# ayushpradhan-dev/robust-speech-analysis-framework

Measured on AMD Instinct MI355X. Metric: audio-seconds processed/sec (extract+CNN-LSTM fwd), higher is better.
Workload: dtype f32

## Files before the change

### robust_speech_analysis_framework_amd/csrc/gemm_f16x3.hip

```cpp
#include <algorithm>
#include <type_traits>

#include "gemm_f16x3.h"

namespace rsaf {

using f32x16 = __attribute__((ext_vector_type(16))) float;
using f16x8 = __attribute__((ext_vector_type(8))) _Float16;
typedef __attribute__((address_space(3))) void* lds_ptr3;
typedef const __attribute__((address_space(1))) void* glb_ptr3;

__device__ __forceinline__ unsigned short f16_bits(_Float16 h) { return __builtin_bit_cast(unsigned short, h); }

__device__ __forceinline__ void split2(float xs, unsigned short& h, unsigned short& l) {
    const _Float16 hh = (_Float16)xs;
    const _Float16 ll = (_Float16)(xs - (float)hh);
    h = f16_bits(hh);
    l = f16_bits(ll);
}

template <int TM_, int TN_, int WM_, int WN_, int NST_, int WGS_>
struct H3Cfg {
    static constexpr int TM = TM_, TN = TN_, WM = WM_, WN = WN_, NST = NST_, WGS = WGS_;
    static constexpr int BM = 32 * TM * WM, BN = 32 * TN * WN, BK = 16, NPL = 2;
    static constexpr int THREADS = 64 * WM * WN;
    static constexpr int A_PLANE = BM * BK, B_PLANE = BN * BK;
    static constexpr int STAGE = NPL * (A_PLANE + B_PLANE);
    static constexpr int A_INSTR = BM / 32, B_INSTR = BN / 32;
    static constexpr int PATCH_BYTES = WM * WN * 32 * 36 * 4;
    static constexpr int TAB_BYTES = 2 * (BM + BN) * 4 + 2 * BM * 4;
    static constexpr bool PATCH_IN_STAGE2 = BM > 256;
    static_assert(!PATCH_IN_STAGE2 || STAGE * 2 >= PATCH_BYTES, "stage 2 must hold the epilogue patches");
    static constexpr int LDS_BYTES = NST * STAGE * 2 + (PATCH_IN_STAGE2 ? 0 : PATCH_BYTES) + TAB_BYTES;
};

#if defined(__HIP_DEVICE_COMPILE__)
#define H3_OPAQUE(SP, LB) asm volatile("" : "+s"(SP), "+v"(LB))
#else
#define H3_OPAQUE(SP, LB) (void)0
#endif
#define H3_ADDR(UNIFORM_BASE, LANE_BYTES)                                                                      \
    ({                                                                                                         \
        const char* sp_ = reinterpret_cast<const char*>(UNIFORM_BASE);                                         \
        unsigned lb_ = (LANE_BYTES);                                                                           \
        H3_OPAQUE(sp_, lb_);                                                                                   \
        (glb_ptr3)(sp_ + lb_);                                                                                 \
    })

template <class CFG, int ACT, bool OUT_F32, bool OUT_PLANES, bool HAS_R, bool ROWTAB = false>
__global__ __launch_bounds__(CFG::THREADS, CFG::WGS * CFG::THREADS / 256) void gemm_f16x3_kernel(const GemmH3Params p) {
    extern __shared__ __attribute__((aligned(1024))) unsigned short smem3[];
    constexpr int BM = CFG::BM, BN = CFG::BN, BK = CFG::BK, STAGE = CFG::STAGE, NST = CFG::NST, NPL = CFG::NPL;
    constexpr int TM = CFG::TM, TN = CFG::TN, NW = CFG::WM * CFG::WN;
    constexpr int A_PLANE = CFG::A_PLANE, B_PLANE = CFG::B_PLANE;

    const int tid = threadIdx.x, lane = tid & 63, wave = __builtin_amdgcn_readfirstlane(tid >> 6), l31 = lane & 31, h = lane >> 5;
    const unsigned total_tiles = (unsigned)p.nwg * (unsigned)p.nz;
    const int wm0 = (wave / CFG::WN) * (32 * TM), wn0 = (wave % CFG::WN) * (32 * TN);

    struct Tile { int m0, n0, Mz, z, z1, z2; int64_t coff, aoff, boff; unsigned t; bool valid; };
    auto next_valid = [&](unsigned t) {
        Tile T;
        T.valid = false;
        for (; t < total_tiles; t += gridDim.x) {
            const H3Tile W = h3_tile_at(p, (int)t);
            T.m0 = W.tm * BM; T.n0 = W.tn * BN; T.z = W.z; T.z1 = W.z1; T.z2 = W.z2;
            T.Mz = p.ztab ? (int)p.ztab[2 * W.z1] : p.M;
            if (T.m0 < T.Mz) {
                T.coff = p.ztab ? p.ztab[2 * W.z1 + 1] : -1;
                T.aoff = W.z1 * p.sA + W.z2 * p.sA2 + (int64_t)T.m0 * (p.a_panel ? 16 : p.lda);
                T.boff = W.z2 * p.sB2 + (int64_t)T.n0 * (p.b_panel ? 16 : p.ldb);
                T.t = t; T.valid = true;
                break;
            }
        }
        return T;
    };

    constexpr int NI = CFG::A_INSTR + CFG::B_INSTR;
    constexpr int IPW = (NI + NW - 1) / NW;
    constexpr int A_SLOTS = CFG::A_INSTR / NW;
    constexpr int LAST_LIVE = NI - NW * (IPW - 1);
    static_assert(CFG::A_INSTR % NW == 0, "a slot is an A or a B instruction for every wave alike");
    static_assert(LAST_LIVE == NW || LAST_LIVE <= NW / 2, "the waves of group B have the same number of DMA instructions");
    const bool last_live = LAST_LIVE == NW || wave < LAST_LIVE;
#define H3_LIVE(i) ((i) < IPW - 1 || last_live)
    const char* src[IPW][NPL];
    unsigned voff[IPW];
    int ldsoff[IPW];
    int pc = 0;
    const H3KStep a_step = h3_kstep(p.a_panel ? (int64_t)(p.a_panel_rows > 0 ? p.a_panel_rows : p.M) * 16 : 16, p.a_tap_panels, 2);
    const int64_t b_step = 2 * (p.b_panel ? (int64_t)(p.b_panel_rows > 0 ? p.b_panel_rows : p.N) * 16 : 16);
#pragma unroll
    for (int i = 0; i < IPW; ++i) {
        const int jj = i < A_SLOTS ? wave + NW * i : wave + NW * i - CFG::A_INSTR;
        ldsoff[i] = i < A_SLOTS ? jj * 512 : NPL * A_PLANE + jj * 512;
    }
    auto set_tile = [&](const Tile& T) {
        pc = 0;
#pragma unroll
        for (int i = 0; i < IPW; ++i) {
            const bool isA = i < A_SLOTS;
            const int jj = isA ? wave + NW * i : wave + NW * i - CFG::A_INSTR;
            const int row = 32 * jj + (lane >> 1);
            const int dch = (lane & 1) ^ ((row >> 3) & 1);
            const int rr = isA ? ((T.m0 + row < T.Mz) ? row : T.Mz - 1 - T.m0)
                               : ((T.n0 + row < p.N) ? row : p.N - 1 - T.n0);
            const int64_t rs = isA ? (p.a_panel ? 16 : p.lda) : (p.b_panel ? 16 : p.ldb);
            voff[i] = 2u * ((unsigned)rr * (unsigned)rs + 8u * dch);
            const unsigned short* base = isA ? p.A + T.aoff : p.B + T.boff;
#pragma unroll
            for (int pl = 0; pl < NPL; ++pl)
                src[i][pl] = reinterpret_cast<const char*>(base + pl * (isA ? p.a_plane : p.b_plane));
        }
    };
#define H3_DMA(ST)                                                                                              \
    do {                                                                                                        \
        _Pragma("unroll") for (int i = 0; i < IPW; ++i) {                                                       \
            if (H3_LIVE(i)) {                                                                                   \
                _Pragma("unroll") for (int pl = 0; pl < NPL; ++pl)                                              \
                    __builtin_amdgcn_global_load_lds(H3_ADDR(src[i][pl], voff[i]),                              \
                        (lds_ptr3)(smem3 + (ST) + ldsoff[i] + pl * (i < A_SLOTS ? A_PLANE : B_PLANE)), 16, 0, 0); \
            }                                                                                                   \
        }                                                                                                       \
    } while (0)
#define H3_ADVANCE()                                                                                            \
    do {                                                                                                        \
        const int64_t a_inc_ = h3_kstep_next(a_step, pc);                                                       \
        _Pragma("unroll") for (int i = 0; i < IPW; ++i)                                                         \
            _Pragma("unroll") for (int pl = 0; pl < NPL; ++pl) src[i][pl] += i < A_SLOTS ? a_inc_ : b_step;     \
    } while (0)
    const int nk = p.K / BK;
    auto prefetch = [&](const Tile& T) {
        set_tile(T);
        H3_DMA(0);
        if (nk > 1) {
            H3_ADVANCE();
            H3_DMA(STAGE);
            H3_ADVANCE();
        }
    };

    static_assert(NST == 3 && TM % 2 == 0, "the staggered loop needs three stages and an even number of m-tiles");
    const int grpB = wave >= NW / 2 ? 1 : 0;
    constexpr int NDMA_B = NPL * (LAST_LIVE == NW ? IPW : IPW - 1);
    constexpr int HM = TM / 2;
    constexpr int PATCH_LD = 36;
    float* patch = reinterpret_cast<float*>(smem3 + (CFG::PATCH_IN_STAGE2 ? 2 : NST) * STAGE) + wave * (32 * PATCH_LD);

    constexpr int TPT = (BM + BN + CFG::THREADS - 1) / CFG::THREADS;
    float* tab0 = reinterpret_cast<float*>(smem3 + NST * STAGE) + (CFG::PATCH_IN_STAGE2 ? 0 : NW * (32 * PATCH_LD));
    float* tab1 = tab0 + (BM + BN);
    int* tab_slot = reinterpret_cast<int*>(tab1 + (BM + BN));
    int* tab_dest = tab_slot + BM;
    float e0[TPT], e1[TPT];
    int e_slot[TPT], e_dest[TPT];
    auto load_epi = [&](const Tile& T) {
#pragma unroll
        for (int u = 0; u < TPT; ++u) {
            const int i = tid + u * CFG::THREADS;
            e0[u] = 1.0f; e1[u] = 0.0f;
            if (i < BM) {
                const int row = T.m0 + i < T.Mz ? T.m0 + i : T.Mz - 1;
                if (ROWTAB) {
                    const int2 rt = reinterpret_cast<const int2*>(p.row_tab)[row];
                    e_slot[u] = rt.x; e_dest[u] = rt.y;
                    e0[u] = p.a_scale[rt.x];
                    e1[u] = (OUT_PLANES && p.Cp) ? p.c_scale[rt.x] : 1.0f;
                } else {
                    e0[u] = p.a_scale[(int64_t)T.z1 * p.a_scale_zs + (int64_t)row * p.a_scale_ms];
                    e1[u] = (OUT_PLANES && p.Cp) ? p.c_scale[(int64_t)T.z1 * p.c_scale_zs + (int64_t)row * p.c_scale_ms] : 1.0f;
                }
            } else if (i < BM + BN) {
                const int col = T.n0 + i - BM;
                e0[u] = col < p.N ? p.b_scale[T.z2 * p.sBias2 + col] : 1.0f;
                e1[u] = (p.bias && col < p.N) ? p.bias[T.z2 * p.sBias2 + col] : 0.0f;
            }
        }
    };
    Tile cur = next_valid(blockIdx.x);
    if (!cur.valid) return;
    load_epi(cur);
    prefetch(cur);

    while (true) {
    const Tile nxt = next_valid(cur.t + gridDim.x);
    f32x16 acc[TM][TN];
#pragma unroll
    for (int i = 0; i < TM; ++i)
#pragma unroll
        for (int j = 0; j < TN; ++j)
#pragma unroll
            for (int e = 0; e < 16; ++e) acc[i][j][e] = 0.0f;

    int s0 = 0, s1 = STAGE, s2 = 2 * STAGE;
    auto ktile = [&](auto refill_c, auto grpb_c) __attribute__((always_inline)) {
        constexpr bool REFILL = decltype(refill_c)::value, GRPB = decltype(grpb_c)::value;
        if (!GRPB) asm volatile("s_waitcnt vmcnt(0)" ::: "memory");
        __builtin_amdgcn_s_barrier();
        asm volatile("" ::: "memory");
        const unsigned short* img = smem3 + s0;
        f16x8 bf[TN][NPL];
#pragma unroll
        for (int nt = 0; nt < TN; ++nt) {
            const int row = wn0 + nt * 32 + l31;
            const int off = row * BK + ((h ^ ((row >> 3) & 1)) << 3);
#pragma unroll
            for (int pl = 0; pl < NPL; ++pl) bf[nt][pl] = *reinterpret_cast<const f16x8*>(&img[NPL * A_PLANE + pl * B_PLANE + off]);
        }
        if (REFILL) {
            H3_DMA(GRPB ? s2 : s1);
            H3_ADVANCE();
        }
        f16x8 afp[NPL];
#pragma unroll
        for (int mt = 0; mt < TM; ++mt) {
            f16x8 af[NPL];
            if (mt == HM) {
#pragma unroll
                for (int pl = 0; pl < NPL; ++pl) af[pl] = afp[pl];
            } else {
                const int row = wm0 + mt * 32 + l31;
                const int off = row * BK + ((h ^ ((row >> 3) & 1)) << 3);
#pragma unroll
                for (int pl = 0; pl < NPL; ++pl) af[pl] = *reinterpret_cast<const f16x8*>(&img[pl * A_PLANE + off]);
            }
            if (mt == HM - 1) {
                const int row = wm0 + HM * 32 + l31;
                const int off = row * BK + ((h ^ ((row >> 3) & 1)) << 3);
#pragma unroll
                for (int pl = 0; pl < NPL; ++pl) afp[pl] = *reinterpret_cast<const f16x8*>(&img[pl * A_PLANE + off]);
            }
#pragma unroll
            for (int nt = 0; nt < TN; ++nt) {
                f32x16 c = acc[mt][nt];
                c = __builtin_amdgcn_mfma_f32_32x32x16_f16(af[1], bf[nt][0], c, 0, 0, 0);
                c = __builtin_amdgcn_mfma_f32_32x32x16_f16(af[0], bf[nt][1], c, 0, 0, 0);
                c = __builtin_amdgcn_mfma_f32_32x32x16_f16(af[0], bf[nt][0], c, 0, 0, 0);
                acc[mt][nt] = c;
            }
            if (mt == HM - 1) {
                if (GRPB) asm volatile("s_waitcnt vmcnt(%0)" ::"n"(REFILL ? NDMA_B : 0) : "memory");
                __builtin_amdgcn_s_barrier();
                asm volatile("" ::: "memory");
            }
        }
        const int s_ = s0; s0 = s1; s1 = s2; s2 = s_;
    };
    constexpr std::true_type YES{};
    constexpr std::false_type NO{};
    asm volatile("s_waitcnt vmcnt(0)" ::: "memory");
    if (!grpB) {
        ktile(NO, NO);
        for (int kt = 1; kt < nk - 1; ++kt) ktile(YES, NO);
        if (nk > 1) ktile(NO, NO);
        __builtin_amdgcn_s_barrier();
    } else {
        __builtin_amdgcn_s_barrier();
        for (int kt = 0; kt < nk - 2; ++kt) ktile(YES, YES);
        if (nk > 1) ktile(NO, YES);
        ktile(NO, YES);
    }

    const Tile done = cur;
    constexpr int CW = (OUT_PLANES && !OUT_F32) ? 8 : 4, LPR = 32 / CW, RPI = 64 / LPR, NQ = 32 / RPI;
    const int lr = lane / LPR, c4 = CW * (lane % LPR);
    float4 r4[4];
    auto load_r = [&](int mt, int nt) {
        const int tn = done.n0 + wn0 + nt * 32, tm = done.m0 + wm0 + mt * 32;
        const float* Rt = p.R + (int64_t)done.z * p.sR + (int64_t)tm * p.ldr + tn + c4;
#pragma unroll
        for (int q = 0; q < 4; ++q) {
            const bool ok = (tn + c4) < p.N && (tm + 8 * q + lr) < done.Mz;
            r4[q] = (ok && p.R) ? *reinterpret_cast<const float4*>(Rt + (8 * q + lr) * (int)p.ldr) : make_float4(0.f, 0.f, 0.f, 0.f);
        }
    };
#pragma unroll
    for (int u = 0; u < TPT; ++u) {
        const int i = tid + u * CFG::THREADS;
        if (i < BM + BN) { tab0[i] = e0[u]; tab1[i] = e1[u]; }
        if (ROWTAB && i < BM) { tab_slot[i] = e_slot[u]; tab_dest[i] = e_dest[u]; }
    }
    if (HAS_R) load_r(0, 0);

    __syncthreads();
    cur = nxt;
    if (cur.valid) {
        prefetch(cur);
        load_epi(cur);
    }

    {
    const int m0 = done.m0, n0 = done.n0, Mz = done.Mz;
    const int64_t z = done.z, z1 = done.z1, z2 = done.z2;
    static_assert(!HAS_R || CW == 4, "the residual comes with the fp32 output");
#pragma unroll
    for (int mt = 0; mt < TM; ++mt) {
        const int tm = m0 + wm0 + mt * 32;
        float asi[NQ], csc[NQ], row_amax[NQ];
        int drow[NQ];
#pragma unroll
        for (int q = 0; q < NQ; ++q) {
            asi[q] = p.alpha * pow2_inverse(tab0[wm0 + mt * 32 + RPI * q + lr]);
            csc[q] = tab1[wm0 + mt * 32 + RPI * q + lr];
            row_amax[q] = 0.0f;
            drow[q] = ROWTAB ? tab_dest[wm0 + mt * 32 + RPI * q + lr] : tm + RPI * q + lr;
        }
#pragma unroll
        for (int nt = 0; nt < TN; ++nt) {
            const int tn = n0 + wn0 + nt * 32;
            const int gc = tn + c4;
            const bool c_ok = gc < p.N;
            float bsi[CW], bias4[CW];
#pragma unroll
            for (int j4 = 0; j4 < CW / 4; ++j4) {
                const float4 bs4 = *reinterpret_cast<const float4*>(tab0 + BM + wn0 + nt * 32 + c4 + 4 * j4);
                const float4 bi4 = *reinterpret_cast<const float4*>(tab1 + BM + wn0 + nt * 32 + c4 + 4 * j4);
                bsi[4 * j4] = pow2_inverse(bs4.x); bsi[4 * j4 + 1] = pow2_inverse(bs4.y);
                bsi[4 * j4 + 2] = pow2_inverse(bs4.z); bsi[4 * j4 + 3] = pow2_inverse(bs4.w);
                bias4[4 * j4] = bi4.x; bias4[4 * j4 + 1] = bi4.y; bias4[4 * j4 + 2] = bi4.z; bias4[4 * j4 + 3] = bi4.w;
            }
            constexpr int LAST = TM * TN - 1;
            const int sub = mt * TN + nt;
#pragma unroll
            for (int e = 0; e < 16; ++e) patch[(4 * h + (e & 3) + 8 * (e >> 2)) * PATCH_LD + l31] = acc[mt][nt][e];
            __builtin_amdgcn_fence(__ATOMIC_RELEASE, "wavefront");
            __builtin_amdgcn_wave_barrier();
            __builtin_amdgcn_fence(__ATOMIC_ACQUIRE, "wavefront");
            float v[NQ][CW];
#pragma unroll
            for (int q = 0; q < NQ; ++q)
#pragma unroll
                for (int j4 = 0; j4 < CW / 4; ++j4) {
                    const float4 t4 = *reinterpret_cast<const float4*>(patch + (RPI * q + lr) * PATCH_LD + c4 + 4 * j4);
                    v[q][4 * j4] = t4.x; v[q][4 * j4 + 1] = t4.y; v[q][4 * j4 + 2] = t4.z; v[q][4 * j4 + 3] = t4.w;
                }
            __builtin_amdgcn_wave_barrier();
#pragma unroll
            for (int q = 0; q < NQ; ++q) {
                float rv[4] = {0.f, 0.f, 0.f, 0.f};
                if (HAS_R) { rv[0] = r4[q % 4].x; rv[1] = r4[q % 4].y; rv[2] = r4[q % 4].z; rv[3] = r4[q % 4].w; }
#pragma unroll
                for (int j = 0; j < CW; ++j) {
                    float y = v[q][j] * (asi[q] * bsi[j]) + bias4[j];
                    if (HAS_R) y += rv[j % 4];
                    if (ACT == ACT_SILU) y = y / (1.0f + expf(-y));
                    v[q][j] = y;
                    if (ACT == ACT_GELU && (j & 1)) {
                        const gelu_f32x2 g2 = gelu_pair(gelu_f32x2{v[q][j - 1], v[q][j]});
                        v[q][j - 1] = g2.x; v[q][j] = g2.y;
                    }
                    if (ACT != ACT_NONE && (j & 3) == 3) __builtin_amdgcn_sched_barrier(0);
                }
            }
            if (HAS_R && sub < LAST) load_r((sub + 1) / TN, (sub + 1) % TN);
#pragma unroll
            for (int q = 0; q < NQ; ++q) {
                const int row = drow[q];
                const bool ok = c_ok && tm + RPI * q + lr < Mz && (!ROWTAB || row >= 0);
                if (p.amax_out && ok && gc >= p.amax_col_min) {
#pragma unroll
                    for (int j = 0; j < CW; ++j) row_amax[q] = fmaxf(row_amax[q], fabsf(v[q][j]));
                }
                if (ok) {
                    if (OUT_F32 && p.C) *reinterpret_cast<float4*>(p.C + (done.coff >= 0 ? done.coff : z1 * p.sC) + z2 * p.sC2 + (int64_t)row * p.ldc + gc) =
                        make_float4(v[q][0], v[q][1], v[q][2], v[q][3]);
                    if (OUT_PLANES && p.Cp) {
                        const float cs = csc[q];
                        unsigned short hh[CW], ll[CW];
#pragma unroll
                        for (int j = 0; j < CW; ++j) split2(v[q][j] * cs, hh[j], ll[j]);
                        unsigned short* Pt = p.cp_panel ? p.Cp + (int64_t)(gc >> 4) * ((int64_t)p.M * 16) + (int64_t)row * 16 + (gc & 15)
                                                        : p.Cp + z * p.sCp + (int64_t)row * p.ldcp + gc;
                        if (CW == 8) {
                            *reinterpret_cast<uint4*>(Pt) = make_uint4(hh[0] | ((unsigned)hh[1] << 16), hh[2] | ((unsigned)hh[3] << 16),
                                                                      hh[4 % CW] | ((unsigned)hh[5 % CW] << 16), hh[6 % CW] | ((unsigned)hh[7 % CW] << 16));
                            *reinterpret_cast<uint4*>(Pt + p.c_plane) = make_uint4(ll[0] | ((unsigned)ll[1] << 16), ll[2] | ((unsigned)ll[3] << 16),
                                                                                  ll[4 % CW] | ((unsigned)ll[5 % CW] << 16), ll[6 % CW] | ((unsigned)ll[7 % CW] << 16));
                        } else {
                            *reinterpret_cast<uint2*>(Pt) = make_uint2(hh[0] | ((unsigned)hh[1] << 16), hh[2] | ((unsigned)hh[3] << 16));
                            *reinterpret_cast<uint2*>(Pt + p.c_plane) = make_uint2(ll[0] | ((unsigned)ll[1] << 16), ll[2] | ((unsigned)ll[3] << 16));
                        }
                    }
                }
            }
        }
        if (p.amax_out) {
#pragma unroll
            for (int q = 0; q < NQ; ++q) {
                const int row = tm + RPI * q + lr;
                const bool r_ok = row < Mz && (!ROWTAB || drow[q] >= 0);
                const int slot = !r_ok ? -1 : ROWTAB ? tab_slot[wm0 + mt * 32 + RPI * q + lr]
                                                     : (int)(z1 * p.amax_zs) + (p.amax_row_slot ? p.amax_row_slot[row] : 0);
                unsigned long long todo = __ballot(r_ok);
                while (todo) {
                    const int first = __ffsll((long long)todo) - 1;
                    const int s0 = __shfl(slot, first, 64);
                    const bool mine = r_ok && slot == s0;
                    float mx = mine ? row_amax[q] : 0.0f;
#pragma unroll
                    for (int o = 32; o >= 1; o >>= 1) mx = fmaxf(mx, __shfl_xor(mx, o, 64));
                    if (lane == first && mx > 0.0f) atomicMax(p.amax_out + s0, __float_as_uint(mx));
                    todo &= ~__ballot(mine);
                }
            }
        }
    }
    }
    if (!cur.valid) break;
    }
#undef H3_DMA
#undef H3_ADVANCE
#undef H3_LIVE
}

__global__ __launch_bounds__(256) void f16x2_row_scales_kernel(const float* __restrict__ src, int64_t rows, int K, int64_t ld,
                                                               float* __restrict__ scale, float* __restrict__ norm2,
                                                               unsigned* __restrict__ stat_max) {
    const int64_t row = (int64_t)blockIdx.x * 4 + (threadIdx.x >> 6);
    if (row >= rows) return;
    const int lane = threadIdx.x & 63;
    const float* x = src + row * ld;
    float mx = 0.0f;
    double ss = 0.0;
    for (int k = lane; k < K; k += 64) {
        const float v = x[k];
        mx = fmaxf(mx, fabsf(v));
        ss += (double)v * (double)v;
    }
#pragma unroll
    for (int o = 32; o >= 1; o >>= 1) mx = fmaxf(mx, __shfl_xor(mx, o, 64));
    ss = wave_sum_f64(ss);
    if (lane == 0) {
        scale[row] = f16x2_scale_for_bound(mx);
        const float nn = (float)sqrt(ss) * 1.0000002f;
        if (norm2) norm2[row] = nn;
        if (stat_max) {
            atomicMax(stat_max + 0, __float_as_uint(nn));
            atomicMax(stat_max + 1, __float_as_uint(mx));
        }
    }
}

__global__ __launch_bounds__(256) void split_f16x2_kernel(const float* __restrict__ src, int64_t rows, int K, int64_t ld,
                                                          const float* __restrict__ scale, int scale_stride,
                                                          unsigned short* __restrict__ planes, int64_t plane_stride, int panels) {
    const int64_t row = (int64_t)blockIdx.x * 256 + threadIdx.x;
    if (row >= rows) return;
    const int kb = blockIdx.y;
    const float s = scale[row * scale_stride];
    const float4* s4 = reinterpret_cast<const float4*>(src + row * ld + 16 * kb);
    unsigned short h[16], l[16];
#pragma unroll
    for (int q = 0; q < 4; ++q) {
        const float4 v = s4[q];
        split2(v.x * s, h[4 * q], l[4 * q]); split2(v.y * s, h[4 * q + 1], l[4 * q + 1]);
        split2(v.z * s, h[4 * q + 2], l[4 * q + 2]); split2(v.w * s, h[4 * q + 3], l[4 * q + 3]);
    }
    auto pk = [](const unsigned short* s_, int o) {
        return make_uint4(s_[o] | ((unsigned)s_[o + 1] << 16), s_[o + 2] | ((unsigned)s_[o + 3] << 16),
                          s_[o + 4] | ((unsigned)s_[o + 5] << 16), s_[o + 6] | ((unsigned)s_[o + 7] << 16));
    };
    unsigned short* d = panels ? planes + (int64_t)kb * rows * 16 + row * 16 : planes + row * K + 16 * kb;
    *reinterpret_cast<uint4*>(d) = pk(h, 0); *reinterpret_cast<uint4*>(d + 8) = pk(h, 8);
    *reinterpret_cast<uint4*>(d + plane_stride) = pk(l, 0); *reinterpret_cast<uint4*>(d + plane_stride + 8) = pk(l, 8);
}

__global__ __launch_bounds__(256) void scale_from_bound_kernel(const unsigned* __restrict__ amax_bits, int64_t n,
                                                               const float* __restrict__ factor_dev, float factor_host,
                                                               const float* __restrict__ add_dev, float* __restrict__ scale) {
    const int64_t i = (int64_t)blockIdx.x * 256 + threadIdx.x;
    if (i >= n) return;
    const float f = factor_host * (factor_dev ? *factor_dev : 1.0f);
    const float a = add_dev ? *add_dev : 0.0f;
    scale[i] = f16x2_scale_for_bound(__uint_as_float(amax_bits[i]) * f + a);
}

int launch_f16x2_row_scales(const float* src, int64_t rows, int K, int64_t ld, float* scale, float* norm2, unsigned* stat_max,
                            hipStream_t stream) {
    RSAF_CHECK_ARG(rows >= 0 && K >= 0 && ld >= K, "bad shape");
    if (rows == 0) return RSAF_OK;
    RSAF_CHECK_ARG(src && scale, "NULL pointer");
    RSAF_CHECK_ARG((rows + 3) / 4 <= 0x7fffffffLL, "too many rows");
    hipLaunchKernelGGL(f16x2_row_scales_kernel, dim3((unsigned)((rows + 3) / 4)), dim3(256), 0, stream, src, rows, K, ld, scale, norm2,
                       stat_max);
    RSAF_CHECK_HIP(hipGetLastError());
    return RSAF_OK;
}

int launch_split_f16x2(const float* src, int64_t rows, int K, int64_t ld, const float* scale, int scale_stride, uint16_t* planes,
                       int64_t plane_stride, int panels, hipStream_t stream) {
    RSAF_CHECK_ARG(rows >= 0 && K >= 0 && K % 16 == 0 && ld % 4 == 0 && ld >= K, "K must be a non-negative multiple of 16, ld a multiple of 4");
    if (rows == 0 || K == 0) return RSAF_OK;
    RSAF_CHECK_ARG(src && planes && scale, "NULL pointer");
    RSAF_CHECK_ARG(plane_stride % 8 == 0 && K / 16 <= 65535 && (scale_stride == 0 || scale_stride == 1),
                   "plane stride must be a multiple of 8 elements; at most 65535 panels; scale stride 0 or 1");
    RSAF_CHECK_ARG((reinterpret_cast<uintptr_t>(src) & 15) == 0 && (reinterpret_cast<uintptr_t>(planes) & 15) == 0, "16-byte alignment");
    ProfScope prof("split_f16x2", stream, 0.0, 8.0 * (double)rows * K);
    hipLaunchKernelGGL(split_f16x2_kernel, dim3((unsigned)((rows + 255) / 256), (unsigned)(K / 16)), dim3(256), 0, stream, src, rows, K,
                       ld, scale, scale_stride, reinterpret_cast<unsigned short*>(planes), plane_stride, panels);
    RSAF_CHECK_HIP(hipGetLastError());
    return RSAF_OK;
}

int launch_scale_from_bound(const unsigned* amax_bits, int64_t n, const float* factor_dev, float factor_host, const float* add_dev,
                            float* scale, hipStream_t stream) {
    if (n <= 0) return RSAF_OK;
    RSAF_CHECK_ARG(amax_bits && scale, "NULL pointer");
    hipLaunchKernelGGL(scale_from_bound_kernel, dim3((unsigned)((n + 255) / 256)), dim3(256), 0, stream, amax_bits, n, factor_dev,
                       factor_host, add_dev, scale);
    RSAF_CHECK_HIP(hipGetLastError());
    return RSAF_OK;
}

int launch_gemm_f16x3(const GemmH3Params& p, hipStream_t stream, const char* tag) {
    RSAF_CHECK_ARG(p.M >= 0 && p.N >= 0 && p.K >= 0 && p.nz >= 0, "negative dimension");
    if (p.M == 0 || p.N == 0 || p.nz == 0) return RSAF_OK;
    RSAF_CHECK_ARG(p.A && p.B && (p.C || p.Cp), "NULL operand");
    RSAF_CHECK_ARG(p.a_scale && p.b_scale && (!p.Cp || p.c_scale), "every plane operand needs its scales");
    RSAF_CHECK_ARG(p.K % 16 == 0 && p.K >= 16, "K must be a positive multiple of 16");
    RSAF_CHECK_ARG(p.N % 16 == 0, "N must be a multiple of 16 (16-byte epilogue stores)");
    RSAF_CHECK_ARG(p.ldc % 8 == 0 && p.ldcp % 8 == 0 && p.ldr % 4 == 0 && p.c_plane % 8 == 0 && p.sC % 4 == 0 && p.sCp % 8 == 0 &&
                   p.sR % 4 == 0 && p.sC2 % 4 == 0, "ldc / ldr / output strides must keep 16-byte alignment");
    RSAF_CHECK_ARG(p.lda % 8 == 0 && p.ldb % 8 == 0 && p.a_plane % 8 == 0 && p.b_plane % 8 == 0 && p.sA % 8 == 0 && p.sA2 % 8 == 0 &&
                   p.sB2 % 8 == 0, "lda, ldb, the plane strides and the batch strides must be multiples of 8 elements");
    RSAF_CHECK_ARG((reinterpret_cast<uintptr_t>(p.A) & 15) == 0 && (reinterpret_cast<uintptr_t>(p.B) & 15) == 0 &&
                   (reinterpret_cast<uintptr_t>(p.b_scale) & 15) == 0 && p.sBias2 % 4 == 0, "A, B and b_scale must be 16-byte aligned");
    RSAF_CHECK_ARG(!p.R || p.ldr > 0, "residual needs ldr");
    RSAF_CHECK_ARG(p.act >= 0 && p.act <= 2, "act must be 0 (none), 1 (gelu) or 2 (silu)");
    RSAF_CHECK_ARG(p.nz <= 65535, "at most 65535 batches per launch");
    RSAF_CHECK_ARG(!p.cp_panel || p.nz == 1, "the panel layout of the plane output is for unbatched operands");
    RSAF_CHECK_ARG(!p.a_panel || p.nz == 1 || p.a_panel_rows > 0, "a batched A in panels needs a_panel_rows");
    RSAF_CHECK_ARG(p.a_tap_panels == 0 || (p.a_panel && p.a_panel_rows > 0 && p.a_tap_panels > 0 && (p.K / 16) % p.a_tap_panels == 0),
                   "a_tap_panels: A in panels with a_panel_rows, K = taps x a_tap_panels x 16");
    RSAF_CHECK_ARG(p.ldc < (1 << 24) && p.ldcp < (1 << 24) && p.ldr < (1 << 24), "leading dimensions must be below 2^24");
    RSAF_CHECK_ARG(!p.R || p.C, "the residual comes with the fp32 output");
    RSAF_CHECK_ARG(!p.row_tab || (p.nz == 1 && !p.ztab && p.nz2 <= 1 && !p.cp_panel && !p.a_panel && !p.amax_row_slot),
                   "a row table: one batch, row-major A and plane output, no ztab / amax_row_slot");
    RSAF_CHECK_ARG(p.nz2 <= 1 || (p.C && !p.Cp && !p.R && (!p.a_panel || p.a_panel_rows > 0) && p.nz % p.nz2 == 0),
                   "two-level batches: fp32 output only, no residual, A row-major or panels with a_panel_rows, nz a multiple of nz2");
    ProfScope prof(tag ? tag : "gemm_f16x3", stream, 2.0 * p.M * (double)p.N * p.K * p.nz, 0.0);
    using CfgA = H3Cfg<4, 2, 2, 4, 3, 1>;
    using CfgN = H3Cfg<2, 1, 4, 2, 3, 1>;
    using CfgM = H3Cfg<4, 2, 4, 2, 3, 1>;
#define H3_LAUNCH_CFG(CFG, ACT, F32, PL, HR, ...)                                                                       \
    do {                                                                                                                \
        RSAF_CHECK_HIP(hipFuncSetAttribute((const void*)gemm_f16x3_kernel<CFG, ACT, F32, PL, HR, ##__VA_ARGS__>,         \
                                           hipFuncAttributeMaxDynamicSharedMemorySize, CFG::LDS_BYTES));                 \
        RSAF_CHECK_ARG(h3_grid_fill(pp, CFG::BM, CFG::BN), "too many tiles");                                           \
        const int64_t tiles = (int64_t)pp.nwg * pp.nz;                                                                  \
        hipLaunchKernelGGL((gemm_f16x3_kernel<CFG, ACT, F32, PL, HR, ##__VA_ARGS__>),                                    \
                           dim3((unsigned)std::min<int64_t>(tiles, persistent_wgs)), dim3(CFG::THREADS), CFG::LDS_BYTES, stream, pp); \
    } while (0)
#define H3_LAUNCH(ACT, F32, PL, HR, ...)                                                                                \
    do {                                                                                                                \
        if (p.N <= 64) H3_LAUNCH_CFG(CfgN, ACT, F32, PL, HR, ##__VA_ARGS__);                                             \
        else H3_LAUNCH_CFG(CfgA, ACT, F32, PL, HR, ##__VA_ARGS__);                                                       \
    } while (0)
#define H3_LAUNCH3(ACT, F32, PL, HR)                                                                                    \
    do {                                                                                                                \
        if (p.N <= 64) H3_LAUNCH_CFG(CfgN, ACT, F32, PL, HR);                                                            \
        else if (p.N <= 128) H3_LAUNCH_CFG(CfgM, ACT, F32, PL, HR);                                                      \
        else H3_LAUNCH_CFG(CfgA, ACT, F32, PL, HR);                                                                      \
    } while (0)
    GemmH3Params pp = p;
    if (pp.group_m <= 0) pp.group_m = 2;
    int persistent_wgs = 256;
    {
        int dev = 0, cus = 0;
        if (hipGetDevice(&dev) == hipSuccess && hipDeviceGetAttribute(&cus, hipDeviceAttributeMultiprocessorCount, dev) == hipSuccess && cus > 0)
            persistent_wgs = cus;
    }
    const bool f32o = p.C != nullptr, plo = p.Cp != nullptr, hr = p.R != nullptr;
    if (p.row_tab) {
        if (p.act == ACT_GELU && !f32o && plo && !hr) H3_LAUNCH(ACT_GELU, false, true, false, true);
        else if (p.act == ACT_GELU && f32o && !plo && !hr) H3_LAUNCH(ACT_GELU, true, false, false, true);
        else {
            set_error("launch_gemm_f16x3: a row table comes with GELU and one output (planes or fp32)");
            return RSAF_ERR_ARG;
        }
    } else if (p.act == ACT_NONE && f32o && !plo && !hr) H3_LAUNCH3(ACT_NONE, true, false, false);
    else if (p.act == ACT_NONE && f32o && !plo && hr) H3_LAUNCH(ACT_NONE, true, false, true);
    else if (p.act == ACT_GELU && !f32o && plo && !hr) H3_LAUNCH3(ACT_GELU, false, true, false);
    else if (p.act == ACT_SILU && !f32o && plo && !hr) H3_LAUNCH3(ACT_SILU, false, true, false);
    else if (p.act == ACT_GELU && f32o && !plo && !hr) H3_LAUNCH(ACT_GELU, true, false, false);
    else if (p.act == ACT_SILU && f32o && !plo && !hr) H3_LAUNCH(ACT_SILU, true, false, false);
    else if (p.act == ACT_GELU && f32o && !plo && hr) H3_LAUNCH3(ACT_GELU, true, false, true);
    else if (p.act == ACT_SILU && f32o && !plo && hr) H3_LAUNCH3(ACT_SILU, true, false, true);
    else if (p.act == ACT_NONE && !f32o && plo && !hr) H3_LAUNCH(ACT_NONE, false, true, false);
    else if (p.act == ACT_NONE && f32o && plo && !hr) H3_LAUNCH(ACT_NONE, true, true, false);
    else {
        set_error("launch_gemm_f16x3: unsupported combination of activation / outputs / residual");
        return RSAF_ERR_ARG;
    }
#undef H3_LAUNCH_CFG
#undef H3_LAUNCH
#undef H3_LAUNCH3
    RSAF_CHECK_HIP(hipGetLastError());
    return RSAF_OK;
}

}

using namespace rsaf;

extern "C" int rsaf_f16x2_row_scales(const float* src, int64_t rows, int K, int64_t ld, float* scale, float* norm2,
                                     rsaf_stream_t stream) {
    return launch_f16x2_row_scales(src, rows, K, ld, scale, norm2, nullptr, (hipStream_t)stream);
}

extern "C" int rsaf_split_f16x2(const float* src, int64_t rows, int K, int64_t ld, const float* scale, int scale_stride,
                                uint16_t* planes, int64_t plane_stride, int panels, rsaf_stream_t stream) {
    return launch_split_f16x2(src, rows, K, ld, scale, scale_stride, planes, plane_stride, panels, (hipStream_t)stream);
}

extern "C" int rsaf_gemm_f16x3(const uint16_t* A_planes, int64_t a_plane_stride, const float* a_scale, int a_scale_stride,
                               const uint16_t* B_planes, int64_t b_plane_stride, const float* b_scale, float* C,
                               uint16_t* C_planes, int64_t c_plane_stride, const float* c_scale, int c_scale_stride,
                               uint32_t* amax_out, const float* bias, const float* R, int M, int N, int K, int64_t lda, int64_t ldb,
                               int64_t ldc, int64_t ldr, int act, float alpha, int a_panels, int b_panels, int c_panels,
                               rsaf_stream_t stream) {
    GemmH3Params p{};
    p.A = A_planes; p.a_plane = a_plane_stride; p.lda = a_panels ? 16 : lda; p.sA = 0;
    p.a_scale = a_scale; p.a_scale_zs = 0; p.a_scale_ms = a_scale_stride;
    p.B = B_planes; p.b_plane = b_plane_stride; p.ldb = b_panels ? 16 : ldb; p.b_scale = b_scale;
    p.C = C; p.ldc = ldc; p.sC = 0;
    p.Cp = C_planes; p.c_plane = c_plane_stride; p.ldcp = c_panels ? 16 : ldc; p.sCp = 0;
    p.c_scale = c_scale; p.c_scale_zs = 0; p.c_scale_ms = c_scale_stride;
    p.amax_out = amax_out; p.amax_zs = 0; p.amax_row_slot = nullptr; p.amax_col_min = 0;
    p.bias = bias; p.R = R; p.ldr = ldr; p.sR = 0;
    p.M = M; p.N = N; p.K = K; p.nz = 1; p.act = act; p.alpha = alpha;
    p.a_panel = a_panels != 0; p.b_panel = b_panels != 0; p.cp_panel = c_panels != 0;
    return launch_gemm_f16x3(p, (hipStream_t)stream, "gemm_f16x3");
}
```

Baseline: 12370.

## Specialize GEMM epilogue on compile-time traits and precompute destination addressing

Adds an EPI bitmask template parameter (panel layout, amax, row slots, column minimum, ragged ztab, second batch dim) so runtime branches in the epilogue and tile lookup are resolved at compile time. Per-lane destination bases and offsets are precomputed once per tile, and pow2_inverse and alpha are folded into the LDS scale table instead of being recomputed per fragment. This is meant to cut epilogue integer address arithmetic and register pressure. In exchange it creates a large explicit list of instantiations, and any trait combination not listed now fails with an error.

```diff
diff --git a/robust_speech_analysis_framework_amd/csrc/gemm_f16x3.hip b/robust_speech_analysis_framework_amd/csrc/gemm_f16x3.hip
--- a/robust_speech_analysis_framework_amd/csrc/gemm_f16x3.hip
+++ b/robust_speech_analysis_framework_amd/csrc/gemm_f16x3.hip
@@ -47,8 +47,21 @@
         (glb_ptr3)(sp_ + lb_);                                                                                 \
     })
 
-template <class CFG, int ACT, bool OUT_F32, bool OUT_PLANES, bool HAS_R, bool ROWTAB = false>
+enum : unsigned {
+    EPI_PANEL = 1,
+    EPI_AMAX = 2,
+    EPI_ROW_SLOT = 4,
+    EPI_COL_MIN = 8,
+    EPI_RAGGED = 16,
+    EPI_NZ2 = 32,
+};
+
+template <class CFG, int ACT, bool OUT_F32, bool OUT_PLANES, bool HAS_R, bool ROWTAB, unsigned EPI>
 __global__ __launch_bounds__(CFG::THREADS, CFG::WGS * CFG::THREADS / 256) void gemm_f16x3_kernel(const GemmH3Params p) {
+    constexpr bool PANEL = (EPI & EPI_PANEL) != 0, AMAX = (EPI & EPI_AMAX) != 0, ROW_SLOT = (EPI & EPI_ROW_SLOT) != 0;
+    constexpr bool COL_MIN = (EPI & EPI_COL_MIN) != 0, RAGGED = (EPI & EPI_RAGGED) != 0, NZ2 = (EPI & EPI_NZ2) != 0;
+    static_assert(!PANEL || (OUT_PLANES && !ROWTAB), "panels are a layout of the plane output");
+    static_assert(AMAX || !(ROW_SLOT || COL_MIN), "row slots and the column limit belong to amax_out");
     extern __shared__ __attribute__((aligned(1024))) unsigned short smem3[];
     constexpr int BM = CFG::BM, BN = CFG::BN, BK = CFG::BK, STAGE = CFG::STAGE, NST = CFG::NST, NPL = CFG::NPL;
     constexpr int TM = CFG::TM, TN = CFG::TN, NW = CFG::WM * CFG::WN;
@@ -64,12 +77,12 @@
         T.valid = false;
         for (; t < total_tiles; t += gridDim.x) {
             const H3Tile W = h3_tile_at(p, (int)t);
-            T.m0 = W.tm * BM; T.n0 = W.tn * BN; T.z = W.z; T.z1 = W.z1; T.z2 = W.z2;
-            T.Mz = p.ztab ? (int)p.ztab[2 * W.z1] : p.M;
+            T.m0 = W.tm * BM; T.n0 = W.tn * BN; T.z = W.z; T.z1 = NZ2 ? W.z1 : W.z; T.z2 = NZ2 ? W.z2 : 0;
+            T.Mz = RAGGED ? (int)p.ztab[2 * T.z1] : p.M;
             if (T.m0 < T.Mz) {
-                T.coff = p.ztab ? p.ztab[2 * W.z1 + 1] : -1;
-                T.aoff = W.z1 * p.sA + W.z2 * p.sA2 + (int64_t)T.m0 * (p.a_panel ? 16 : p.lda);
-                T.boff = W.z2 * p.sB2 + (int64_t)T.n0 * (p.b_panel ? 16 : p.ldb);
+                T.coff = (RAGGED && OUT_F32) ? p.ztab[2 * T.z1 + 1] : -1;
+                T.aoff = T.z1 * p.sA + (NZ2 ? T.z2 * p.sA2 : 0) + (int64_t)T.m0 * (p.a_panel ? 16 : p.lda);
+                T.boff = (NZ2 ? T.z2 * p.sB2 : 0) + (int64_t)T.n0 * (p.b_panel ? 16 : p.ldb);
                 T.t = t; T.valid = true;
                 break;
             }
@@ -166,10 +179,10 @@
                     const int2 rt = reinterpret_cast<const int2*>(p.row_tab)[row];
                     e_slot[u] = rt.x; e_dest[u] = rt.y;
                     e0[u] = p.a_scale[rt.x];
-                    e1[u] = (OUT_PLANES && p.Cp) ? p.c_scale[rt.x] : 1.0f;
+                    e1[u] = OUT_PLANES ? p.c_scale[rt.x] : 1.0f;
                 } else {
                     e0[u] = p.a_scale[(int64_t)T.z1 * p.a_scale_zs + (int64_t)row * p.a_scale_ms];
-                    e1[u] = (OUT_PLANES && p.Cp) ? p.c_scale[(int64_t)T.z1 * p.c_scale_zs + (int64_t)row * p.c_scale_ms] : 1.0f;
+                    e1[u] = OUT_PLANES ? p.c_scale[(int64_t)T.z1 * p.c_scale_zs + (int64_t)row * p.c_scale_ms] : 1.0f;
                 }
             } else if (i < BM + BN) {
                 const int col = T.n0 + i - BM;
@@ -265,20 +278,45 @@
     const Tile done = cur;
     constexpr int CW = (OUT_PLANES && !OUT_F32) ? 8 : 4, LPR = 32 / CW, RPI = 64 / LPR, NQ = 32 / RPI;
     const int lr = lane / LPR, c4 = CW * (lane % LPR);
+    const int wm = done.m0 + wm0, wn = done.n0 + wn0;
+    const int rows_left = done.Mz - wm - lr, cols_left = p.N - wn - c4;
+    struct Dest { char* base; unsigned lane; int64_t row_step, nt_step; };
+    auto dest_rows = [&](const void* origin, int64_t ld, int esz) {
+        Dest d;
+        d.base = reinterpret_cast<char*>(const_cast<void*>(origin)) + ((ROWTAB ? 0 : (int64_t)wm * ld) + wn) * esz;
+        d.lane = ((ROWTAB ? 0u : (unsigned)lr * (unsigned)ld) + (unsigned)c4) * (unsigned)esz;
+        d.row_step = ROWTAB ? ld * esz : RPI * ld * esz;
+        d.nt_step = 32 * esz;
+        return d;
+    };
+    Dest dC{}, dR{}, dP{};
+    if (OUT_F32) dC = dest_rows(p.C + (done.coff >= 0 ? done.coff : done.z1 * p.sC) + (NZ2 ? done.z2 * p.sC2 : 0), p.ldc, 4);
+    if (HAS_R) dR = dest_rows(p.R + (int64_t)done.z * p.sR, p.ldr, 4);
+    if (OUT_PLANES && !PANEL) dP = dest_rows(p.Cp + (int64_t)done.z * p.sCp, p.ldcp, 2);
+    if (PANEL) {
+        const int64_t panel = (int64_t)p.M * 32;
+        dP.base = reinterpret_cast<char*>(p.Cp) + (wn >> 4) * panel + (int64_t)wm * 32;
+        dP.lane = (unsigned)(c4 >> 4) * (unsigned)panel + 32u * lr + 2u * (c4 & 15);
+        dP.row_step = RPI * 32;
+        dP.nt_step = 2 * panel;
+    }
+    const int64_t c_plane_bytes = 2 * p.c_plane;
+    auto dest_at = [&](const Dest& d, int i, int nt, int drow) {
+        return ROWTAB ? d.base + (int64_t)drow * d.row_step + d.lane + nt * d.nt_step
+                      : d.base + (i * d.row_step + nt * d.nt_step) + d.lane;
+    };
     float4 r4[4];
     auto load_r = [&](int mt, int nt) {
-        const int tn = done.n0 + wn0 + nt * 32, tm = done.m0 + wm0 + mt * 32;
-        const float* Rt = p.R + (int64_t)done.z * p.sR + (int64_t)tm * p.ldr + tn + c4;
 #pragma unroll
         for (int q = 0; q < 4; ++q) {
-            const bool ok = (tn + c4) < p.N && (tm + 8 * q + lr) < done.Mz;
-            r4[q] = (ok && p.R) ? *reinterpret_cast<const float4*>(Rt + (8 * q + lr) * (int)p.ldr) : make_float4(0.f, 0.f, 0.f, 0.f);
+            const bool ok = 32 * nt < cols_left && 32 * mt + 8 * q < rows_left;
+            r4[q] = ok ? *reinterpret_cast<const float4*>(dest_at(dR, mt * 4 + q, nt, 0)) : make_float4(0.f, 0.f, 0.f, 0.f);
         }
     };
 #pragma unroll
     for (int u = 0; u < TPT; ++u) {
         const int i = tid + u * CFG::THREADS;
-        if (i < BM + BN) { tab0[i] = e0[u]; tab1[i] = e1[u]; }
+        if (i < BM + BN) { tab0[i] = i < BM ? p.alpha * pow2_inverse(e0[u]) : pow2_inverse(e0[u]); tab1[i] = e1[u]; }
         if (ROWTAB && i < BM) { tab_slot[i] = e_slot[u]; tab_dest[i] = e_dest[u]; }
     }
     if (HAS_R) load_r(0, 0);
@@ -291,33 +329,29 @@
     }
 
     {
-    const int m0 = done.m0, n0 = done.n0, Mz = done.Mz;
-    const int64_t z = done.z, z1 = done.z1, z2 = done.z2;
     static_assert(!HAS_R || CW == 4, "the residual comes with the fp32 output");
 #pragma unroll
     for (int mt = 0; mt < TM; ++mt) {
-        const int tm = m0 + wm0 + mt * 32;
         float asi[NQ], csc[NQ], row_amax[NQ];
         int drow[NQ];
+        bool row_ok[NQ];
 #pragma unroll
         for (int q = 0; q < NQ; ++q) {
-            asi[q] = p.alpha * pow2_inverse(tab0[wm0 + mt * 32 + RPI * q + lr]);
+            asi[q] = tab0[wm0 + mt * 32 + RPI * q + lr];
             csc[q] = tab1[wm0 + mt * 32 + RPI * q + lr];
             row_amax[q] = 0.0f;
-            drow[q] = ROWTAB ? tab_dest[wm0 + mt * 32 + RPI * q + lr] : tm + RPI * q + lr;
+            drow[q] = ROWTAB ? tab_dest[wm0 + mt * 32 + RPI * q + lr] : 0;
+            row_ok[q] = 32 * mt + RPI * q < rows_left && (!ROWTAB || drow[q] >= 0);
         }
 #pragma unroll
         for (int nt = 0; nt < TN; ++nt) {
-            const int tn = n0 + wn0 + nt * 32;
-            const int gc = tn + c4;
-            const bool c_ok = gc < p.N;
+            const bool c_ok = 32 * nt < cols_left;
             float bsi[CW], bias4[CW];
 #pragma unroll
             for (int j4 = 0; j4 < CW / 4; ++j4) {
                 const float4 bs4 = *reinterpret_cast<const float4*>(tab0 + BM + wn0 + nt * 32 + c4 + 4 * j4);
                 const float4 bi4 = *reinterpret_cast<const float4*>(tab1 + BM + wn0 + nt * 32 + c4 + 4 * j4);
-                bsi[4 * j4] = pow2_inverse(bs4.x); bsi[4 * j4 + 1] = pow2_inverse(bs4.y);
-                bsi[4 * j4 + 2] = pow2_inverse(bs4.z); bsi[4 * j4 + 3] = pow2_inverse(bs4.w);
+                bsi[4 * j4] = bs4.x; bsi[4 * j4 + 1] = bs4.y; bsi[4 * j4 + 2] = bs4.z; bsi[4 * j4 + 3] = bs4.w;
                 bias4[4 * j4] = bi4.x; bias4[4 * j4 + 1] = bi4.y; bias4[4 * j4 + 2] = bi4.z; bias4[4 * j4 + 3] = bi4.w;
             }
             constexpr int LAST = TM * TN - 1;
@@ -356,42 +390,38 @@
             if (HAS_R && sub < LAST) load_r((sub + 1) / TN, (sub + 1) % TN);
 #pragma unroll
             for (int q = 0; q < NQ; ++q) {
-                const int row = drow[q];
-                const bool ok = c_ok && tm + RPI * q + lr < Mz && (!ROWTAB || row >= 0);
-                if (p.amax_out && ok && gc >= p.amax_col_min) {
+                const bool ok = c_ok && row_ok[q];
+                if (AMAX && ok && (!COL_MIN || wn + 32 * nt + c4 >= p.amax_col_min)) {
 #pragma unroll
                     for (int j = 0; j < CW; ++j) row_amax[q] = fmaxf(row_amax[q], fabsf(v[q][j]));
                 }
                 if (ok) {
-                    if (OUT_F32 && p.C) *reinterpret_cast<float4*>(p.C + (done.coff >= 0 ? done.coff : z1 * p.sC) + z2 * p.sC2 + (int64_t)row * p.ldc + gc) =
-                        make_float4(v[q][0], v[q][1], v[q][2], v[q][3]);
-                    if (OUT_PLANES && p.Cp) {
+                    if (OUT_F32) *reinterpret_cast<float4*>(dest_at(dC, mt * NQ + q, nt, drow[q])) = make_float4(v[q][0], v[q][1], v[q][2], v[q][3]);
+                    if (OUT_PLANES) {
                         const float cs = csc[q];
                         unsigned short hh[CW], ll[CW];
 #pragma unroll
                         for (int j = 0; j < CW; ++j) split2(v[q][j] * cs, hh[j], ll[j]);
-                        unsigned short* Pt = p.cp_panel ? p.Cp + (int64_t)(gc >> 4) * ((int64_t)p.M * 16) + (int64_t)row * 16 + (gc & 15)
-                                                        : p.Cp + z * p.sCp + (int64_t)row * p.ldcp + gc;
+                        char* Pt = dest_at(dP, mt * NQ + q, nt, drow[q]);
                         if (CW == 8) {
                             *reinterpret_cast<uint4*>(Pt) = make_uint4(hh[0] | ((unsigned)hh[1] << 16), hh[2] | ((unsigned)hh[3] << 16),
                                                                       hh[4 % CW] | ((unsigned)hh[5 % CW] << 16), hh[6 % CW] | ((unsigned)hh[7 % CW] << 16));
-                            *reinterpret_cast<uint4*>(Pt + p.c_plane) = make_uint4(ll[0] | ((unsigned)ll[1] << 16), ll[2] | ((unsigned)ll[3] << 16),
-                                                                                  ll[4 % CW] | ((unsigned)ll[5 % CW] << 16), ll[6 % CW] | ((unsigned)ll[7 % CW] << 16));
+                            *reinterpret_cast<uint4*>(Pt + c_plane_bytes) = make_uint4(ll[0] | ((unsigned)ll[1] << 16), ll[2] | ((unsigned)ll[3] << 16),
+                                                                                      ll[4 % CW] | ((unsigned)ll[5 % CW] << 16), ll[6 % CW] | ((unsigned)ll[7 % CW] << 16));
                         } else {
                             *reinterpret_cast<uint2*>(Pt) = make_uint2(hh[0] | ((unsigned)hh[1] << 16), hh[2] | ((unsigned)hh[3] << 16));
-                            *reinterpret_cast<uint2*>(Pt + p.c_plane) = make_uint2(ll[0] | ((unsigned)ll[1] << 16), ll[2] | ((unsigned)ll[3] << 16));
+                            *reinterpret_cast<uint2*>(Pt + c_plane_bytes) = make_uint2(ll[0] | ((unsigned)ll[1] << 16), ll[2] | ((unsigned)ll[3] << 16));
                         }
                     }
                 }
             }
         }
-        if (p.amax_out) {
+        if (AMAX) {
 #pragma unroll
             for (int q = 0; q < NQ; ++q) {
-                const int row = tm + RPI * q + lr;
-                const bool r_ok = row < Mz && (!ROWTAB || drow[q] >= 0);
+                const bool r_ok = row_ok[q];
                 const int slot = !r_ok ? -1 : ROWTAB ? tab_slot[wm0 + mt * 32 + RPI * q + lr]
-                                                     : (int)(z1 * p.amax_zs) + (p.amax_row_slot ? p.amax_row_slot[row] : 0);
+                                                     : (int)(done.z1 * p.amax_zs) + (ROW_SLOT ? p.amax_row_slot[wm + 32 * mt + RPI * q + lr] : 0);
                 unsigned long long todo = __ballot(r_ok);
                 while (todo) {
                     const int first = __ffsll((long long)todo) - 1;
@@ -509,6 +539,17 @@
     RSAF_CHECK_ARG(amax_bits && scale, "NULL pointer");
     hipLaunchKernelGGL(scale_from_bound_kernel, dim3((unsigned)((n + 255) / 256)), dim3(256), 0, stream, amax_bits, n, factor_dev,
                        factor_host, add_dev, scale);
+    RSAF_CHECK_HIP(hipGetLastError());
+    return RSAF_OK;
+}
+
+template <class CFG, int ACT, bool OUT_F32, bool OUT_PLANES, bool HAS_R, bool ROWTAB, unsigned EPI>
+static int h3_launch(GemmH3Params& pp, int wgs, hipStream_t stream) {
+    const auto kernel = gemm_f16x3_kernel<CFG, ACT, OUT_F32, OUT_PLANES, HAS_R, ROWTAB, EPI>;
+    RSAF_CHECK_HIP(hipFuncSetAttribute((const void*)kernel, hipFuncAttributeMaxDynamicSharedMemorySize, CFG::LDS_BYTES));
+    RSAF_CHECK_ARG(h3_grid_fill(pp, CFG::BM, CFG::BN), "too many tiles");
+    const int64_t tiles = (int64_t)pp.nwg * pp.nz;
+    hipLaunchKernelGGL(kernel, dim3((unsigned)std::min<int64_t>(tiles, wgs)), dim3(CFG::THREADS), CFG::LDS_BYTES, stream, pp);
     RSAF_CHECK_HIP(hipGetLastError());
     return RSAF_OK;
 }
@@ -534,6 +575,7 @@
     RSAF_CHECK_ARG(p.a_tap_panels == 0 || (p.a_panel && p.a_panel_rows > 0 && p.a_tap_panels > 0 && (p.K / 16) % p.a_tap_panels == 0),
                    "a_tap_panels: A in panels with a_panel_rows, K = taps x a_tap_panels x 16");
     RSAF_CHECK_ARG(p.ldc < (1 << 24) && p.ldcp < (1 << 24) && p.ldr < (1 << 24), "leading dimensions must be below 2^24");
+    RSAF_CHECK_ARG(!p.cp_panel || p.M < (1 << 26), "the panel layout of the plane output takes fewer than 2^26 rows");
     RSAF_CHECK_ARG(!p.R || p.C, "the residual comes with the fp32 output");
     RSAF_CHECK_ARG(!p.row_tab || (p.nz == 1 && !p.ztab && p.nz2 <= 1 && !p.cp_panel && !p.a_panel && !p.amax_row_slot),
                    "a row table: one batch, row-major A and plane output, no ztab / amax_row_slot");
@@ -543,26 +585,6 @@
     using CfgA = H3Cfg<4, 2, 2, 4, 3, 1>;
     using CfgN = H3Cfg<2, 1, 4, 2, 3, 1>;
     using CfgM = H3Cfg<4, 2, 4, 2, 3, 1>;
-#define H3_LAUNCH_CFG(CFG, ACT, F32, PL, HR, ...)                                                                       \
-    do {                                                                                                                \
-        RSAF_CHECK_HIP(hipFuncSetAttribute((const void*)gemm_f16x3_kernel<CFG, ACT, F32, PL, HR, ##__VA_ARGS__>,         \
-                                           hipFuncAttributeMaxDynamicSharedMemorySize, CFG::LDS_BYTES));                 \
-        RSAF_CHECK_ARG(h3_grid_fill(pp, CFG::BM, CFG::BN), "too many tiles");                                           \
-        const int64_t tiles = (int64_t)pp.nwg * pp.nz;                                                                  \
-        hipLaunchKernelGGL((gemm_f16x3_kernel<CFG, ACT, F32, PL, HR, ##__VA_ARGS__>),                                    \
-                           dim3((unsigned)std::min<int64_t>(tiles, persistent_wgs)), dim3(CFG::THREADS), CFG::LDS_BYTES, stream, pp); \
-    } while (0)
-#define H3_LAUNCH(ACT, F32, PL, HR, ...)                                                                                \
-    do {                                                                                                                \
-        if (p.N <= 64) H3_LAUNCH_CFG(CfgN, ACT, F32, PL, HR, ##__VA_ARGS__);                                             \
-        else H3_LAUNCH_CFG(CfgA, ACT, F32, PL, HR, ##__VA_ARGS__);                                                       \
-    } while (0)
-#define H3_LAUNCH3(ACT, F32, PL, HR)                                                                                    \
-    do {                                                                                                                \
-        if (p.N <= 64) H3_LAUNCH_CFG(CfgN, ACT, F32, PL, HR);                                                            \
-        else if (p.N <= 128) H3_LAUNCH_CFG(CfgM, ACT, F32, PL, HR);                                                      \
-        else H3_LAUNCH_CFG(CfgA, ACT, F32, PL, HR);                                                                      \
-    } while (0)
     GemmH3Params pp = p;
     if (pp.group_m <= 0) pp.group_m = 2;
     int persistent_wgs = 256;
@@ -571,33 +593,49 @@
         if (hipGetDevice(&dev) == hipSuccess && hipDeviceGetAttribute(&cus, hipDeviceAttributeMultiprocessorCount, dev) == hipSuccess && cus > 0)
             persistent_wgs = cus;
     }
-    const bool f32o = p.C != nullptr, plo = p.Cp != nullptr, hr = p.R != nullptr;
-    if (p.row_tab) {
-        if (p.act == ACT_GELU && !f32o && plo && !hr) H3_LAUNCH(ACT_GELU, false, true, false, true);
-        else if (p.act == ACT_GELU && f32o && !plo && !hr) H3_LAUNCH(ACT_GELU, true, false, false, true);
-        else {
-            set_error("launch_gemm_f16x3: a row table comes with GELU and one output (planes or fp32)");
-            return RSAF_ERR_ARG;
-        }
-    } else if (p.act == ACT_NONE && f32o && !plo && !hr) H3_LAUNCH3(ACT_NONE, true, false, false);
-    else if (p.act == ACT_NONE && f32o && !plo && hr) H3_LAUNCH(ACT_NONE, true, false, true);
-    else if (p.act == ACT_GELU && !f32o && plo && !hr) H3_LAUNCH3(ACT_GELU, false, true, false);
-    else if (p.act == ACT_SILU && !f32o && plo && !hr) H3_LAUNCH3(ACT_SILU, false, true, false);
-    else if (p.act == ACT_GELU && f32o && !plo && !hr) H3_LAUNCH(ACT_GELU, true, false, false);
-    else if (p.act == ACT_SILU && f32o && !plo && !hr) H3_LAUNCH(ACT_SILU, true, false, false);
-    else if (p.act == ACT_GELU && f32o && !plo && hr) H3_LAUNCH3(ACT_GELU, true, false, true);
-    else if (p.act == ACT_SILU && f32o && !plo && hr) H3_LAUNCH3(ACT_SILU, true, false, true);
-    else if (p.act == ACT_NONE && !f32o && plo && !hr) H3_LAUNCH(ACT_NONE, false, true, false);
-    else if (p.act == ACT_NONE && f32o && plo && !hr) H3_LAUNCH(ACT_NONE, true, true, false);
-    else {
-        set_error("launch_gemm_f16x3: unsupported combination of activation / outputs / residual");
-        return RSAF_ERR_ARG;
-    }
-#undef H3_LAUNCH_CFG
-#undef H3_LAUNCH
-#undef H3_LAUNCH3
-    RSAF_CHECK_HIP(hipGetLastError());
-    return RSAF_OK;
+    const bool f32o = p.C != nullptr, plo = p.Cp != nullptr, hr = p.R != nullptr, rt = p.row_tab != nullptr;
+    const unsigned epi = (plo && p.cp_panel ? EPI_PANEL : 0u) | (p.amax_out ? EPI_AMAX : 0u) |
+                         (p.amax_out && p.amax_row_slot ? EPI_ROW_SLOT : 0u) | (p.amax_out && p.amax_col_min > 0 ? EPI_COL_MIN : 0u) |
+                         (p.ztab ? EPI_RAGGED : 0u) | (p.nz2 > 1 ? EPI_NZ2 : 0u);
+#define H3_GO(CFG, ...) h3_launch<CFG, __VA_ARGS__>(pp, persistent_wgs, stream)
+#define H3_NA(...) return p.N <= 64 ? H3_GO(CfgN, __VA_ARGS__) : H3_GO(CfgA, __VA_ARGS__)
+#define H3_NMA(...) return p.N <= 64 ? H3_GO(CfgN, __VA_ARGS__) : p.N <= 128 ? H3_GO(CfgM, __VA_ARGS__) : H3_GO(CfgA, __VA_ARGS__)
+#define H3_A(...) if (p.N > 64) return H3_GO(CfgA, __VA_ARGS__)
+#define H3_CASE(CFGS, ACT, F32, PL, HR, RT, EPI)                                                                        \
+    if (p.act == ACT && f32o == F32 && plo == PL && hr == HR && rt == RT && epi == (EPI)) { H3_##CFGS(ACT, F32, PL, HR, RT, (EPI)); }
+    H3_CASE(NA,  ACT_GELU, false, true,  false, true,  EPI_AMAX)
+    H3_CASE(NA,  ACT_GELU, true,  false, false, true,  0)
+    H3_CASE(NMA, ACT_NONE, true,  false, false, false, 0)
+    H3_CASE(NMA, ACT_NONE, true,  false, false, false, EPI_AMAX)
+    H3_CASE(NMA, ACT_NONE, true,  false, false, false, EPI_AMAX | EPI_ROW_SLOT)
+    H3_CASE(NMA, ACT_NONE, true,  false, false, false, EPI_RAGGED)
+    H3_CASE(NA,  ACT_NONE, true,  false, true,  false, 0)
+    H3_CASE(NA,  ACT_NONE, true,  false, true,  false, EPI_AMAX)
+    H3_CASE(NA,  ACT_NONE, false, true,  false, false, 0)
+    H3_CASE(A,   ACT_NONE, false, true,  false, false, EPI_PANEL)
+    H3_CASE(A,   ACT_NONE, false, true,  false, false, EPI_AMAX)
+    H3_CASE(A,   ACT_NONE, false, true,  false, false, EPI_PANEL | EPI_AMAX)
+    H3_CASE(NA,  ACT_NONE, true,  true,  false, false, EPI_AMAX)
+    H3_CASE(NA,  ACT_NONE, true,  true,  false, false, EPI_PANEL | EPI_AMAX)
+    H3_CASE(NMA, ACT_GELU, false, true,  false, false, EPI_PANEL)
+    H3_CASE(NMA, ACT_GELU, false, true,  false, false, EPI_AMAX)
+    H3_CASE(NA,  ACT_GELU, false, true,  false, false, EPI_PANEL | EPI_AMAX)
+    H3_CASE(A,   ACT_GELU, false, true,  false, false, 0)
+    H3_CASE(NMA, ACT_SILU, false, true,  false, false, EPI_AMAX)
+    H3_CASE(NA,  ACT_GELU, true,  false, false, false, EPI_AMAX)
+    H3_CASE(NA,  ACT_GELU, true,  false, false, false, EPI_RAGGED | EPI_NZ2)
+    H3_CASE(NA,  ACT_SILU, true,  false, false, false, EPI_AMAX)
+    H3_CASE(NMA, ACT_GELU, true,  false, true,  false, EPI_AMAX)
+    H3_CASE(NMA, ACT_SILU, true,  false, true,  false, EPI_AMAX)
+#undef H3_CASE
+#undef H3_A
+#undef H3_NMA
+#undef H3_NA
+#undef H3_GO
+    set_error("launch_gemm_f16x3: no instantiation for act " + std::to_string(p.act) + ", fp32 output " + std::to_string(f32o) +
+              ", plane output " + std::to_string(plo) + ", residual " + std::to_string(hr) + ", row table " + std::to_string(rt) +
+              ", epilogue traits " + std::to_string(epi) + (p.N <= 64 ? ", N <= 64" : ""));
+    return RSAF_ERR_ARG;
 }
 
 }
```

New measurement: 12490 (median of 6 runs). Within noise of the previous version (+0.9%).
